# byu-magicc/VI-EKF

Hardware: AMD Instinct MI355X
Metric: EKF steps/sec (IMU-rate propagate + N_feat updates), batch=1024, N_feat=50 (higher is better)
Workload: dtype f64

## Files before the change

vi_ekf_amd/csrc/viekf_resident_common.hpp:

```cpp
#pragma once
#include <type_traits>

#include "viekf_fused_lds.hpp"
#include "viekf_instance_rows.hpp"
#include "viekf_kernel_args.hpp"

namespace viekf {

#ifndef RES_INLINE
#define RES_INLINE __forceinline__
#endif
__device__ __forceinline__ void wave_lds_sync() {
  __builtin_amdgcn_fence(__ATOMIC_RELEASE, "wavefront");
  __builtin_amdgcn_wave_barrier();
  __builtin_amdgcn_fence(__ATOMIC_ACQUIRE, "wavefront");
}
__device__ __forceinline__ int opaque(int v) { asm volatile("" : "+v"(v)); return v; }
typedef double v2f64 __attribute__((ext_vector_type(2)));
__device__ __forceinline__ double2 lds_ld2(const double* p) {
  const v2f64 v = *reinterpret_cast<const v2f64*>(p);
  return make_double2(v.x, v.y);
}
template <bool ON>
__device__ __forceinline__ void group_fence() {
  if (ON) {
    asm volatile("" ::: "memory");
    __builtin_amdgcn_sched_barrier(0);
  }
}
__device__ __forceinline__ double uniform_f64(double v) {
  const unsigned long long u = __double_as_longlong(v);
  const unsigned lo = __builtin_amdgcn_readfirstlane((unsigned)u), hi = __builtin_amdgcn_readfirstlane((unsigned)(u >> 32));
  return __longlong_as_double(((unsigned long long)hi << 32) | lo);
}

#ifdef VIEKF_STAMPS
#if VIEKF_STAMPS + 0 == 2
#define RES_STAMP_KEPT(idx) ((idx) >= 192 && (idx) < 224)
#else
#define RES_STAMP_KEPT(idx) true
#endif
#define RES_STAMP(S_, who, idx)                                                                  \
  do {                                                                                           \
    if (RES_STAMP_KEPT(idx) && (S_).b == 0 && (who)) {                                                                  \
      __builtin_amdgcn_sched_barrier(0);                                                         \
      reinterpret_cast<unsigned long long*>((S_).stamps)[(idx)] = __builtin_amdgcn_s_memtime();  \
      __builtin_amdgcn_sched_barrier(0);                                                         \
    }                                                                                            \
  } while (0)
#else
#define RES_STAMP(S_, who, idx) do {} while (0)
#endif

#ifdef VIEKF_ISA_MARKS
#define RES_MARK(name)                          \
  do {                                          \
    __builtin_amdgcn_sched_barrier(0);          \
    asm volatile("; @@MARK " name);             \
    __builtin_amdgcn_sched_barrier(0);          \
  } while (0)
#else
#define RES_MARK(name) do {} while (0)
#endif

#ifdef VIEKF_ABLATE
#define RES_ABLATE(S_, bit) (((S_).dbg & (bit)) != 0)
#else
#define RES_ABLATE(S_, bit) false
#endif

typedef __attribute__((address_space(3))) volatile int lds_vint_t;

struct ResShared {
  double *xs, *Kt, *Wt, *Praw, *lam, *sm, *fixadd, *fixset, *Z, *phiff, *Abb, *Gb, *Phibb, *Mbb, *Gdb, *Pbb, *T16,
      *xdb, *Pbc, *PhibbT, *Pd, *PsiP, *Pi, *Xi, *AvG, *Lbc, *mz, *mR;
  int* mslot;
  int2* mseq;
  BodyCtx* ctx;
  int N, n, nf, len, M, mstride, do_prop, b, dbg, kp, B, img_len, mcap;
  int fmt;
  long si, so;
  double* stamps;
};

template <int RB, int TW>
__device__ __forceinline__ void res_words(const int* __restrict__ resmap, int t, int (&w)[RB]) {
#pragma unroll
  for (int ia = 0; ia < RB; ia++) w[ia] = resmap[ia * TW + t];
}
constexpr bool res_setup_under_load(int RB, int NW, bool MP) {
  return res_batched_loads(RB, NW) && !MP && ((NW == 3 && (RB == 4 || RB == 6 || RB == 7)) || (NW == 6 && RB == 5));
}
#ifndef VIEKF_SERVICE_SETUP
#define VIEKF_SERVICE_SETUP 1
#endif
#ifndef VIEKF_SERVICE_SETUP_CHUNKS
#define VIEKF_SERVICE_SETUP_CHUNKS 1
#endif
constexpr bool res_service_setup(int RB, int NW, bool MP) {
  return (VIEKF_SERVICE_SETUP) != 0 && res_setup_under_load(RB, NW, MP) && RB != 4;
}
#ifndef VIEKF_ROTATING_READS
#define VIEKF_ROTATING_READS 3
#endif
constexpr int res_rotating_reads(int RB, int NW, bool MP, bool ZU) {
  return (RB > 4) ? ((VIEKF_ROTATING_READS) & 3) : 0;
}
__device__ __forceinline__ bool res_word_blk(int e, int& I, int& J) {
  I = e & 0xff;
  J = (e >> 8) & 0xff;
  return (e >> 16) != 0;
}

__device__ __forceinline__ int res_next_valid(const ResShared& S, int from) {
  int m = from;
  while (m < S.M && S.mslot[m] < 0) m++;
  return m;
}

}
```

vi_ekf_amd/csrc/viekf_resident_worker.hpp:

```cpp
#pragma once
#include "viekf_resident_prop.hpp"

namespace viekf {


struct StoreChunk { int f0, f1, rb, h; };
__device__ __forceinline__ bool store_chunk_at(int f0, int N, int n, int img_len, StoreChunk& c) {
  if (f0 >= N) return false;
  c.f0 = f0;
  c.rb = (16 + 3 * f0) & ~1;
  c.h = ((n + 1) & ~1) - c.rb;
  c.f1 = min(N, f0 + max(1, img_len / (3 * c.h)));
  return true;
}
template <int T>
__device__ __forceinline__ void res_store_chunk(const StreamArgs& a, const ResShared& S, const StoreChunk& c, int tid) {
  const int n = S.n, ld = a.ld;
  double* P = a.P_out + S.so * n * ld;
  const double* img = S.Z;
  const int ncol = 3 * (c.f1 - c.f0), lane = tid & 63, w = tid >> 6;
  constexpr int NWV = T / 64;
  if ((n & 1) == 0) {
#pragma unroll 2
    for (int col = w; col < ncol; col += NWV) {
      const int j = 16 + 3 * c.f0 + col;
      const double* src = img + col * c.h - c.rb;
      for (int i0 = c.rb; i0 < n; i0 += 256) {
        double2 v[2];
#pragma unroll
        for (int u = 0; u < 2; u++) v[u] = lds_ld2(src + min(i0 + 2 * (lane + 64 * u), n - 2));
#pragma unroll
        for (int u = 0; u < 2; u++) {
          const int i = i0 + 2 * (lane + 64 * u);
          if (i < n && i + 1 >= j) *reinterpret_cast<double2*>(P + i + (long)j * ld) = v[u];
        }
      }
    }
  } else {
#pragma unroll 2
    for (int col = w; col < ncol; col += NWV) {
      const int j = 16 + 3 * c.f0 + col;
      const double* src = img + col * c.h - c.rb;
      for (int i = c.rb + lane; i < n; i += 64)
        if (i >= j) P[i + (long)j * ld] = src[i];
    }
  }
}

template <int RB, int TW>
__device__ __forceinline__ void res_store_packed(double* img, const double (&pb)[RB][9], const double* Pbc, const double* Pbb,
                                                 int N, int t) {
  constexpr ResPack K(0, RB, TW / 64);
  v2f64* dst = reinterpret_cast<v2f64*>(img) + t;
#pragma unroll
  for (int p = 0; p < K.npair; p++) {
    v2f64 v;
    v.x = pb[(2 * p) / 9][(2 * p) % 9];
    v.y = pb[(2 * p + 1) / 9][(2 * p + 1) % 9];
    dst[p * TW] = v;
  }
  if ((9 * RB) & 1) img[K.single + t] = pb[RB - 1][8];
  v2f64* gc = reinterpret_cast<v2f64*>(img + K.pbc);
  for (int e = t; e < 24 * N; e += TW) gc[e] = *reinterpret_cast<const v2f64*>(Pbc + 2 * e);
  v2f64* gb = reinterpret_cast<v2f64*>(img + K.pbc + 48 * N);
  for (int e = t; e < 128; e += TW) gb[e] = *reinterpret_cast<const v2f64*>(Pbb + 2 * e);
}
__device__ __forceinline__ void res_body_items(const ResShared& S, const double* kP, bool run, int id, int nthreads,
                                               int first, int last, int slot2, double* rawdst) {
  const double* wP = kP + 2 * S.n;
  double* Pbc = S.Pbc;
  const int j2 = ((first + id) & 7) * 2;
  double2 cw0 = {}, cw1 = {}, cl[3] = {};
  if (run) {
    cw0 = lds_ld2(wP + 2 * j2);
    cw1 = lds_ld2(wP + 2 * j2 + 2);
#pragma unroll
    for (int q = 0; q < 3; q++) cl[q] = lds_ld2(S.Lbc + 16 * q + j2);
  }
#pragma unroll 1
  for (int item = first + id; item < last; item += nthreads) {
    const int g = item >> 3;
    double2 cpv[3];
#pragma unroll
    for (int q = 0; q < 3; q++) cpv[q] = lds_ld2(Pbc + (3 * g + q) * 16 + j2);
    if (run) {
      double2 cki[3];
#pragma unroll
      for (int q = 0; q < 3; q++) cki[q] = lds_ld2(kP + 2 * (16 + 3 * g + q));
#pragma unroll
      for (int q = 0; q < 3; q++) {
        cpv[q].x = fma(-cl[q].x, fma(cki[q].y, cw0.y, cki[q].x * cw0.x), cpv[q].x);
        cpv[q].y = fma(-cl[q].y, fma(cki[q].y, cw1.y, cki[q].x * cw1.x), cpv[q].y);
        *reinterpret_cast<double2*>(Pbc + (3 * g + q) * 16 + j2) = cpv[q];
      }
    }
    if (g == slot2) {
      double* st = rawdst + 2 * j2;
      *reinterpret_cast<double2*>(st) = make_double2(cpv[0].x, cpv[1].x);
      *reinterpret_cast<double2*>(st + 2) = make_double2(cpv[0].y, cpv[1].y);
    }
  }
}
template <int RB, int TW, bool MP, int T = TW + 64, bool ZU = false, bool BL = true>
__device__ __forceinline__ void res_worker(const StreamArgs& a, const ResShared& S, int tid) {
  constexpr bool SU = res_setup_under_load(RB, TW / 64, MP);
  constexpr int RR = res_rotating_reads(RB, TW / 64, MP, ZU);
  const int N = S.N, n = S.n, ld = a.ld, nf = S.nf, len = S.len;
  double* P = a.P + S.si * n * ld;
  const int tid_ = tid;
  constexpr int NWV = TW / 64;
  const DevParams& prm = *a.dp;
  double* Pbc = S.Pbc;
  double* Pbb = S.Pbb;
  const int* __restrict__ resmap = a.resmap;
  auto blk = [&](const int (&w)[RB], int t, int ia, int& I, int& J) -> bool {
    return res_word_blk(BL ? w[ia] : resmap[ia * TW + t], I, J);
  };
  const bool own_diag = tid_ < N;

  double pb[RB][9];
  const bool ldp = (S.fmt & RES_FMT_LOAD_PACKED) != 0;
  double Lff[9];
  bool partial_su = false;
  if (SU) {
    const double lf[3] = {a.lambda[16], a.lambda[17], a.lambda[18]};
#pragma unroll
    for (int r = 0; r < 3; r++)
#pragma unroll
      for (int s = 0; s < 3; s++) Lff[r * 3 + s] = uniform_f64(prm.use_partial_update ? (lf[s] + lf[r] - lf[r] * lf[s]) : 1.0);
    partial_su = prm.use_partial_update != 0;
  }
  if (ldp) {
    const int t = opaque(tid_);
    constexpr ResPack K(0, RB, TW / 64);
    const v2f64* gc = reinterpret_cast<const v2f64*>(P + K.pbc);
    for (int e = t; e < 24 * N; e += TW) *reinterpret_cast<v2f64*>(Pbc + 2 * e) = gc[e];
    const v2f64* gb = reinterpret_cast<const v2f64*>(P + K.pbc + 48 * N);
    for (int e = t; e < 128; e += TW) *reinterpret_cast<v2f64*>(Pbb + 2 * e) = gb[e];
  }
  if (SU) {
    for (int e = tid; !ldp && e < nf * 16; e += TW) {
      const int k = e / nf, row = e - k * nf;
      Pbc[row * 16 + k] = P[(16 + row) + (long)k * ld];
    }
    for (int e = tid; !ldp && e < 256; e += TW) {
      const int r = e & 15, c = e >> 4;
      Pbb[r * 16 + c] = P[max(r, c) + (long)min(r, c) * ld];
    }
  }
  int ws[SU ? RB : 1];
  double qs[3];
  {
    const int tq = opaque(tid_);
    int ew[RB];
    if (BL) res_words<RB, TW>(resmap, tq, ew);
    if (SU) {
#pragma unroll
      for (int ia = 0; ia < RB; ia++) ws[ia] = ew[ia];
      if (S.do_prop) {
#pragma unroll
        for (int r = 0; r < 3; r++) qs[r] = a.Qx[16 + 3 * min(tq, N - 1) + r];
      }
    }
#pragma unroll
    for (int ia = 0; ia < (SU ? RB / 4 : RB); ia++) {
      int I, J;
      blk(ew, tq, ia, I, J);
      const bool up = I < J;
      const int br = 16 + 3 * (up ? J : I), bc = 16 + 3 * (up ? I : J);
      const unsigned cbase = (unsigned)(br + bc * ld);
      const unsigned base = ldp ? 2u * (unsigned)tq : cbase, base1 = ldp ? (unsigned)tq : cbase;
#pragma unroll
      for (int s = 0; s < 3; s++)
#pragma unroll
        for (int r = 0; r < 3; r++) {
          const int rr = (I == J) ? max(r, s) : (up ? s : r), cc = (I == J) ? min(r, s) : (up ? r : s);
          constexpr ResPack K(0, RB, TW / 64);
          const int q = ia * 9 + r * 3 + s;
          const unsigned offp = (unsigned)K.elem(q, 0), offc = (unsigned)(rr + cc * ld);
          pb[ia][r * 3 + s] = P[((q < 2 * K.npair) ? base : base1) + (ldp ? offp : offc)];
        }
    }
    for (int e = tid; !SU && !ldp && e < nf * 16; e += TW) {
      const int k = e / nf, row = e - k * nf;
      Pbc[row * 16 + k] = P[(16 + row) + (long)k * ld];
    }
    for (int e = tid; !SU && !ldp && e < 256; e += TW) {
      const int r = e & 15, c = e >> 4;
      Pbb[r * 16 + c] = P[max(r, c) + (long)min(r, c) * ld];
    }
  }

  auto issue_chunk = [&](auto kc) {
    constexpr int k = decltype(kc)::value + 1, lo = RB * k / 4, hi = RB * (k + 1) / 4;
    const int tq = opaque(tid_);
#pragma unroll
    for (int ia = lo; ia < hi; ia++) {
      int I, J;
      res_word_blk(ws[SU ? ia : 0], I, J);
      const bool up = I < J;
      const int br = 16 + 3 * (up ? J : I), bc = 16 + 3 * (up ? I : J);
      const unsigned cbase = (unsigned)(br + bc * ld);
      const unsigned base = ldp ? 2u * (unsigned)tq : cbase, base1 = ldp ? (unsigned)tq : cbase;
#pragma unroll
      for (int s = 0; s < 3; s++)
#pragma unroll
        for (int r = 0; r < 3; r++) {
          const int rr = (I == J) ? max(r, s) : (up ? s : r), cc = (I == J) ? min(r, s) : (up ? r : s);
          constexpr ResPack K(0, RB, TW / 64);
          const int q = ia * 9 + r * 3 + s;
          const unsigned offp = (unsigned)K.elem(q, 0), offc = (unsigned)(rr + cc * ld);
          pb[ia][r * 3 + s] = P[((q < 2 * K.npair) ? base : base1) + (ldp ? offp : offc)];
        }
    }
  };

  auto sym_diag = [&]() {
    if (own_diag) { pb[0][3] = pb[0][1]; pb[0][6] = pb[0][2]; pb[0][7] = pb[0][5]; }
  };
  if (!SU) {
    sym_diag();
    const double lf[3] = {a.lambda[16], a.lambda[17], a.lambda[18]};
#pragma unroll
    for (int r = 0; r < 3; r++)
#pragma unroll
      for (int s = 0; s < 3; s++) Lff[r * 3 + s] = uniform_f64(prm.use_partial_update ? (lf[s] + lf[r] - lf[r] * lf[s]) : 1.0);
  }
  const bool partial = SU ? partial_su : prm.use_partial_update != 0;
  int par = 0;
  constexpr int NSV = (T - TW) / 64;
  auto fix_word = [&](int mb) -> double { return (NSV > 1) ? S.sm[res_sm::fix_word(1, mb)] + S.sm[res_sm::fix_word(2, mb)] : S.sm[res_sm::fix_word(0, mb)]; };
  RES_STAMP(S, tid == 0, 64);
  __syncthreads();
  RES_STAMP(S, tid == 0, 65);

  const int nkp = MP ? S.kp : 1;
  int eu[RB];
  if (S.do_prop)
   for (int kp = 0; kp < nkp; kp++) {
    const int tk = MP ? opaque(tid) : tid;
    const double* Z = S.Z; double* phiff = S.phiff;
    int ep[RB];
    double qd[3];
    if (SU) {
#pragma unroll
      for (int ia = 0; ia < RB; ia++) ep[ia] = ws[SU ? ia : 0];
#pragma unroll
      for (int r = 0; r < 3; r++) qd[r] = qs[r];
    } else if (BL) {
      const int tq = opaque(tid_);
      res_words<RB, TW>(resmap, tq, ep);
#pragma unroll
      for (int r = 0; r < 3; r++) qd[r] = a.Qx[16 + 3 * min(tq, N - 1) + r];
    }
    if (MP || !BL) res_prop_setup<TW>(a, S, tk);
    else if (SU) res_prop_setup<TW, true, decltype(issue_chunk), res_service_setup(RB, TW / 64, MP)>(a, S, tk, issue_chunk);
    else res_prop_setup<TW, true>(a, S, tk);
    RES_STAMP(S, tid == 0, 66);
    __syncthreads();
    RES_STAMP(S, tid == 0, 67);
#ifdef VIEKF_STAMPS
    asm volatile("s_waitcnt vmcnt(0)" ::: "memory");
#endif
    RES_STAMP(S, tid == 0, 74);
    if (SU) sym_diag();

#pragma unroll
    for (int ia = 0; ia < RB; ia++) {
      const int tq = BL ? 0 : opaque(tid_);
      int I, J;
      const bool v = blk(ep, tq, ia, I, J);
      const double* fj = phiff + 9 * J;
#pragma unroll
      for (int r = 0; r < 3; r++) {
        const double p0 = pb[ia][r * 3 + 0], p1 = pb[ia][r * 3 + 1], p2 = pb[ia][r * 3 + 2];
#pragma unroll
        for (int s = 0; s < 3; s++) pb[ia][r * 3 + s] = p0 * fj[s * 3 + 0] + p1 * fj[s * 3 + 1] + p2 * fj[s * 3 + 2];
      }
      const double* fi = phiff + 9 * I;
#pragma unroll
      for (int s = 0; s < 3; s++) {
        const double p0 = pb[ia][0 * 3 + s], p1 = pb[ia][1 * 3 + s], p2 = pb[ia][2 * 3 + s];
#pragma unroll
        for (int r = 0; r < 3; r++) pb[ia][r * 3 + s] = fi[r * 3 + 0] * p0 + fi[r * 3 + 1] * p1 + fi[r * 3 + 2] * p2;
      }
      if (BL) {
        if (ia == 0 && own_diag) { pb[0][0] += qd[0]; pb[0][4] += qd[1]; pb[0][8] += qd[2]; }
      } else if (v && I == J) {
        pb[ia][0] += a.Qx[16 + 3 * I + 0];
        pb[ia][4] += a.Qx[16 + 3 * I + 1];
        pb[ia][8] += a.Qx[16 + 3 * I + 2];
      }
      __builtin_amdgcn_sched_barrier(0);
      if (RB > 4) {
#pragma unroll
        for (int e = 0; e < 9; e++) asm volatile("" : "+v"(pb[ia][e]));
      }
      group_fence<(RB > 4)>();
    }
    RES_STAMP(S, tid == 0, 68);
    int zoff[RB];
    {
      const int tq = BL ? 0 : opaque(tid_);
#pragma unroll
      for (int ia = 0; ia < RB; ia++) {
        int I, J;
        blk(ep, tq, ia, I, J);
        zoff[ia] = (3 * I * ZS) | ((3 * J * ZS) << 16);
      }
    }
    auto contract = [&](int k, auto crossed) {
      constexpr bool CROSS = decltype(crossed)::value;
      if (RR & 2) {
        double2 xb[2][3], yb[2][3];
#pragma unroll
        for (int ia = 0; ia < 2; ia++) {
          const double* zi = Z + (zoff[ia] & 0xffff) + 2 * k;
          const double* zj = Z + (zoff[ia] >> 16) + 2 * k;
#pragma unroll
          for (int r = 0; r < 3; r++) xb[ia][r] = lds_ld2(zi + r * ZS);
#pragma unroll
          for (int s = 0; s < 3; s++) yb[ia][s] = lds_ld2(zj + s * ZS);
        }
#pragma unroll
        for (int ia = 0; ia < RB; ia++) {
          const int ib = ia & 1;
#pragma unroll
          for (int r = 0; r < 3; r++)
#pragma unroll
            for (int s = 0; s < 3; s++) {
              double acc = pb[ia][r * 3 + s];
              acc = fma(xb[ib][r].x, CROSS ? yb[ib][s].y : yb[ib][s].x, acc);
              acc = fma(xb[ib][r].y, CROSS ? yb[ib][s].x : yb[ib][s].y, acc);
              pb[ia][r * 3 + s] = acc;
            }
          group_fence<true>();
          if (ia + 2 < RB) {
            constexpr int RBL = RB - 1;
            const int in = (ia + 2 < RB) ? ia + 2 : RBL;
            const double* zi = Z + (zoff[in] & 0xffff) + 2 * k;
            const double* zj = Z + (zoff[in] >> 16) + 2 * k;
#pragma unroll
            for (int r = 0; r < 3; r++) xb[ib][r] = lds_ld2(zi + r * ZS);
#pragma unroll
            for (int s = 0; s < 3; s++) yb[ib][s] = lds_ld2(zj + s * ZS);
          }
        }
        return;
      }
#pragma unroll
      for (int ia = 0; ia < RB; ia++) {
        const double* zi = Z + (zoff[ia] & 0xffff) + 2 * k;
        const double* zj = Z + (zoff[ia] >> 16) + 2 * k;
        double2 xv[3], yv[3];
#pragma unroll
        for (int r = 0; r < 3; r++) xv[r] = lds_ld2(zi + r * ZS);
#pragma unroll
        for (int s = 0; s < 3; s++) yv[s] = lds_ld2(zj + s * ZS);
#pragma unroll
        for (int r = 0; r < 3; r++)
#pragma unroll
          for (int s = 0; s < 3; s++) {
            double acc = pb[ia][r * 3 + s];
            acc = fma(xv[r].x, CROSS ? yv[s].y : yv[s].x, acc);
            acc = fma(xv[r].y, CROSS ? yv[s].x : yv[s].y, acc);
            pb[ia][r * 3 + s] = acc;
          }
        if (ia & 1) group_fence<(RB > 4)>();
      }
    };
#pragma unroll 1
    for (int k = 0; k < ZK; k++) contract(k, std::true_type{});
#pragma unroll 1
    for (int k = ZK; k < ZK + 3; k++) contract(k, std::false_type{});
    sym_diag();
    RES_STAMP(S, tid == 0, 69);
    if (BL && !MP) res_words<RB, TW>(resmap, opaque(tid_), eu);
    if (MP) res_prop_body<TW, BL>(a, S, tk);
    par ^= 1;
    RES_STAMP(S, tid == 0, 70);
    __syncthreads();
    for (int e = tk; e < 256; e += TW) { const int r = e >> 4, c = e & 15; Pbb[e] = S.Mbb[min(r, c) * 16 + max(r, c)]; }
    if (MP && kp + 1 < nkp && own_diag && tid_ < len && fix_word(par ^ 1) != 0.0) {
      const int mb = par ^ 1, I = tid_;
      const double ad = S.fixadd[mb * N + I], st = S.fixset[mb * N + I];
      if (ad != 0.0) { pb[0][8] += ad; S.fixadd[mb * N + I] = 0.0; }
      if (st != 0.0) { pb[0][8] = prm.P0_feat[2]; S.fixset[mb * N + I] = 0.0; }
    }
   }

  if (SU && !S.do_prop) {
    issue_chunk(std::integral_constant<int, 0>{});
    issue_chunk(std::integral_constant<int, 1>{});
    issue_chunk(std::integral_constant<int, 2>{});
    sym_diag();
  }
  int Ib[RB], Jb[RB];
  bool vb[RB];
  if (BL && (MP || !S.do_prop)) res_words<RB, TW>(resmap, opaque(tid_), eu);
#pragma unroll
  for (int ia = 0; ia < RB; ia++) vb[ia] = blk(eu, tid_, ia, Ib[ia], Jb[ia]);
  const double p0rr = uniform_f64(prm.P0_feat[2]);
  auto bb_mask = [&](int r, int c) -> double { const double lr_ = S.lam[r], lc_ = S.lam[c]; return partial ? (lc_ + lr_ - lr_ * lc_) : 1.0; };
  double bbL0 = 1.0, bbL1 = 1.0;
  {
    constexpr int BBT0 = (TW >= 128) ? 128 : TW;
    const int ib0 = tid - (TW - BBT0);
    if (ib0 >= 0 && ib0 < 128) { bbL0 = bb_mask(ib0 >> 3, (ib0 & 7) * 2); bbL1 = bb_mask(ib0 >> 3, (ib0 & 7) * 2 + 1); }
  }
  auto apply_fixes = [&](int mb, double pending) {
    if (pending == 0.0) return;
    if (own_diag && tid_ < len) {
      VIEKF_COLD_BEGIN();
      const int I = tid_;
      const double ad = S.fixadd[mb * N + I], st = S.fixset[mb * N + I];
      if (ad != 0.0) { pb[0][8] += ad; S.fixadd[mb * N + I] = 0.0; }
      if (st != 0.0) { pb[0][8] = p0rr; S.fixset[mb * N + I] = 0.0; }
      VIEKF_COLD_END();
    }
  };
  auto extract_cols = [&](int slot, double* Pw) {
#pragma unroll
    for (int ia = 0; ia < RB; ia++) {
      const int I = Ib[ia], J = Jb[ia];
      const bool asrow = J == slot;
      const bool ascol = !asrow && I == slot;
      if (vb[ia] && (asrow || ascol)) {
        const int base = 16 + 3 * (asrow ? I : J);
        const double a0 = pb[ia][0], a1 = asrow ? pb[ia][1] : pb[ia][3];
        const double b0 = asrow ? pb[ia][3] : pb[ia][1], b1 = pb[ia][4];
        const double c0 = asrow ? pb[ia][6] : pb[ia][2], c1 = asrow ? pb[ia][7] : pb[ia][5];
        *reinterpret_cast<double2*>(Pw + 2 * (base + 0)) = make_double2(a0, a1);
        *reinterpret_cast<double2*>(Pw + 2 * (base + 1)) = make_double2(b0, b1);
        *reinterpret_cast<double2*>(Pw + 2 * (base + 2)) = make_double2(c0, c1);
      }
    }
  };

  int m = res_next_valid(S, 0);
  if (own_diag) {
    *reinterpret_cast<double2*>(S.Pd + 4 * tid_) = make_double2(pb[0][0], pb[0][1]);
    *reinterpret_cast<double2*>(S.Pd + 4 * tid_ + 2) = make_double2(pb[0][3], pb[0][4]);
  }
  int2 sq = S.mseq[min(m, S.mcap - 1)];
  if (m < S.M) {
    apply_fixes(par ^ 1, fix_word(par ^ 1));
    const int s0 = S.mslot[m];
    extract_cols(s0, S.Praw);
    if (sq.y >= 0) extract_cols(sq.y, S.Praw + 2 * n);
    const int e = opaque(tid);
    if (e < 16) {
      const int sf = (e < 8) ? s0 : sq.y, ijj = (e & 7) * 2;
      if (sf >= 0) {
        const double2 q0 = lds_ld2(Pbc + (3 * sf) * 16 + ijj);
        const double2 q1 = lds_ld2(Pbc + (3 * sf + 1) * 16 + ijj);
        double* d = S.Praw + ((e < 8) ? 0 : 2 * n) + 2 * ijj;
        *reinterpret_cast<double2*>(d) = make_double2(q0.x, q1.x);
        *reinterpret_cast<double2*>(d + 2) = make_double2(q0.y, q1.y);
      }
    }
  }
  RES_STAMP(S, tid == 0, 71);
  __syncthreads();
  __syncthreads();
  int it_ = 0;
  int cnt = 0;
  while (m < S.M) {
    const int mnext = sq.x;
    RES_MARK("worker.phase_top");
    const double* kP = (cnt & 1) ? S.Z : S.Kt;
    const double* wP = kP + 2 * n;
    __builtin_amdgcn_s_setprio(1);
    const double fixpending = fix_word(par ^ 1);
    const double gflag = S.sm[res_sm::gate_word(cnt)];
    const double nanw = (NSV > 1) ? S.sm[res_sm::nan_word(1, cnt)] + S.sm[res_sm::nan_word(2, cnt)] : S.sm[res_sm::nan_word(0, cnt)];
    sq = S.mseq[min(mnext, S.mcap - 1)];
    RES_STAMP(S, tid == 0 && it_ < 8, 80 + 4 * it_ + 1);
    RES_STAMP(S, (tid & 63) == 0 && it_ == 3, 192 + 4 * (tid >> 6) + 0);
    const int it = tid;
    constexpr int GB = (RB <= 4) ? RB : 2;
    RES_MARK("worker.block_sweep");
    const bool gated = gflag != 0.0;
    const bool run = !gated && nanw == 0.0 && !RES_ABLATE(S, 1);
    bool fixed = false;
    if (RR & 1) {
      apply_fixes(par ^ 1, fixpending);
      if (run) {
        double2 kb[2][3], wb[2][3];
#pragma unroll
        for (int ia = 0; ia < 2; ia++) {
#pragma unroll
          for (int r = 0; r < 3; r++) kb[ia][r] = lds_ld2(kP + 2 * (16 + 3 * Ib[ia] + r));
#pragma unroll
          for (int s = 0; s < 3; s++) wb[ia][s] = lds_ld2(wP + 2 * (16 + 3 * Jb[ia] + s));
        }
#pragma unroll
        for (int ia = 0; ia < RB; ia++) {
          const int ib = ia & 1;
#pragma unroll
          for (int r = 0; r < 3; r++)
#pragma unroll
            for (int s = 0; s < 3; s++) {
              if (ZU && !(r == 2 && s == 2)) {
                pb[ia][r * 3 + s] = fma(-kb[ib][r].y, wb[ib][s].y, fma(-kb[ib][r].x, wb[ib][s].x, pb[ia][r * 3 + s]));
              } else {
                const double t = fma(kb[ib][r].y, wb[ib][s].y, kb[ib][r].x * wb[ib][s].x);
                pb[ia][r * 3 + s] = fma(-Lff[r * 3 + s], t, pb[ia][r * 3 + s]);
              }
            }
          group_fence<true>();
          if (ia + 2 < RB) {
            constexpr int RBL = RB - 1;
            const int in = (ia + 2 < RB) ? ia + 2 : RBL;
#pragma unroll
            for (int r = 0; r < 3; r++) kb[ib][r] = lds_ld2(kP + 2 * (16 + 3 * Ib[in] + r));
#pragma unroll
            for (int s = 0; s < 3; s++) wb[ib][s] = lds_ld2(wP + 2 * (16 + 3 * Jb[in] + s));
          }
        }
      }
    } else
#pragma unroll
    for (int g0 = 0; g0 < RB; g0 += GB) {
      double2 kI[GB][3], wJ[GB][3];
#pragma unroll
      for (int ig = 0; ig < GB; ig++) {
        const int ia = (g0 + ig < RB) ? g0 + ig : RB - 1;
#pragma unroll
        for (int r = 0; r < 3; r++) kI[ig][r] = lds_ld2(kP + 2 * (16 + 3 * Ib[ia] + r));
#pragma unroll
        for (int s = 0; s < 3; s++) wJ[ig][s] = lds_ld2(wP + 2 * (16 + 3 * Jb[ia] + s));
      }
      if (!fixed) { apply_fixes(par ^ 1, fixpending); fixed = true; }
      if (run) {
#pragma unroll
        for (int ig = 0; ig < GB; ig++) {
          if (g0 + ig >= RB) continue;
          const int ia = g0 + ig;
#pragma unroll
          for (int r = 0; r < 3; r++)
#pragma unroll
            for (int s = 0; s < 3; s++) {
              if (ZU && !(r == 2 && s == 2)) {
                pb[ia][r * 3 + s] = fma(-kI[ig][r].y, wJ[ig][s].y, fma(-kI[ig][r].x, wJ[ig][s].x, pb[ia][r * 3 + s]));
              } else {
                const double t = fma(kI[ig][r].y, wJ[ig][s].y, kI[ig][r].x * wJ[ig][s].x);
                pb[ia][r * 3 + s] = fma(-Lff[r * 3 + s], t, pb[ia][r * 3 + s]);
              }
            }
        }
      }
      group_fence<(RB > GB)>();
    }
    sym_diag();
    RES_MARK("worker.column_extraction");
    RES_STAMP(S, tid == 0 && it_ < 8, 160 + 4 * it_ + 0);
    double* rawdst = S.Praw + (cnt & 1) * 2 * n;
    if (sq.y >= 0 && !RES_ABLATE(S, 4) && !(RES_ABLATE(S, 8) && (cnt & 1))) extract_cols(sq.y, rawdst);
    __builtin_amdgcn_s_setprio(0);
    RES_STAMP(S, tid == 0 && it_ < 8, 160 + 4 * it_ + 1);
    RES_STAMP(S, (tid & 63) == 0 && it_ == 3, 192 + 4 * (tid >> 6) + 2);
    __builtin_amdgcn_sched_barrier(0);
    RES_MARK("worker.body_items");
    res_body_items(S, kP, run, (it >= 64) ? it - 64 : it + TW - 64, TW, 0, 8 * N, sq.y, rawdst);
    RES_MARK("worker.body_block");
    if (run) {
      constexpr int BBT = (TW >= 128) ? 128 : TW;
#pragma unroll
      for (int ib = it - (TW - BBT); ib >= 0 && ib < 128; ib += BBT) {
        const int br = ib >> 3, bc2 = (ib & 7) * 2;
        double2 bpv = *reinterpret_cast<double2*>(Pbb + br * 16 + bc2);
        const double2 kr = lds_ld2(kP + 2 * br), wr = lds_ld2(wP + 2 * br);
        const double2 k0 = lds_ld2(kP + 2 * bc2), w0 = lds_ld2(wP + 2 * bc2);
        const double2 k1 = lds_ld2(kP + 2 * bc2 + 2), w1 = lds_ld2(wP + 2 * bc2 + 2);
        const double L0 = (BBT == 128) ? bbL0 : bb_mask(br, bc2), L1 = (BBT == 128) ? bbL1 : bb_mask(br, bc2 + 1);
        const bool up0 = br <= bc2, up1 = br <= bc2 + 1;
        const double2 ka = up0 ? kr : k0, wa = up0 ? w0 : wr;
        const double2 kb = up1 ? kr : k1, wb = up1 ? w1 : wr;
        bpv.x = fma(-L0, fma(ka.y, wa.y, ka.x * wa.x), bpv.x);
        bpv.y = fma(-L1, fma(kb.y, wb.y, kb.x * wb.x), bpv.y);
        *reinterpret_cast<double2*>(Pbb + br * 16 + bc2) = bpv;
      }
    }
    RES_MARK("worker.phase_tail");
    par ^= 1;
    cnt++;
    RES_STAMP(S, tid == 0 && it_ < 8, 80 + 4 * it_ + 2);
    RES_STAMP(S, (tid & 63) == 0 && it_ == 3, 192 + 4 * (tid >> 6) + 1);
    __syncthreads();
    RES_STAMP(S, tid == 0 && it_ < 8, 80 + 4 * it_ + 3);
    RES_STAMP(S, (tid & 63) == 0 && it_ == 3, 192 + 4 * (tid >> 6) + 3);
    it_++;
    m = mnext;
  }
  RES_MARK("worker.loop_end");
  apply_fixes(par ^ 1, fix_word(par ^ 1));
  RES_STAMP(S, tid == 0, 72);
  __syncthreads();

  P = a.P_out + S.so * n * ld;
  if (S.fmt & RES_FMT_STORE_PACKED) {
    res_store_packed<RB, TW>(P, pb, Pbc, Pbb, N, opaque(tid_));
  } else {
    int es[RB];
    if (BL) res_words<RB, TW>(resmap, opaque(tid_), es);
    for (int e = opaque(tid); e < nf * 16; e += TW) {
      const int k = e / nf, row = e - k * nf;
      P[(16 + row) + (long)k * ld] = Pbc[row * 16 + k];
    }
    for (int e = opaque(tid); e < 256; e += TW) P[(e >> 4) + (long)(e & 15) * ld] = Pbb[e];
    double* img = S.Z;
    const int gtid = threadIdx.x;
    RES_STAMP(S, tid == 0, 224);
    StoreChunk sc;
    int ch = 0;
    for (int f0 = 0; store_chunk_at(f0, N, n, S.img_len, sc); f0 = sc.f1, ch++) {
      const int f1 = sc.f1;
      const int tq = BL ? 0 : opaque(tid_);
#pragma unroll
      for (int ia = 0; ia < RB; ia++) {
        int I, J;
        if (blk(es, tq, ia, I, J)) {
          if (I >= J && J >= f0 && J < f1) {
            double* d = img + (3 * (J - f0)) * sc.h + (16 + 3 * I - sc.rb);
#pragma unroll
            for (int s = 0; s < 3; s++)
#pragma unroll
              for (int r = 0; r < 3; r++) d[s * sc.h + r] = pb[ia][r * 3 + s];
          }
          if (I < J && I >= f0 && I < f1) {
            double* d = img + (3 * (I - f0)) * sc.h + (16 + 3 * J - sc.rb);
#pragma unroll
            for (int r = 0; r < 3; r++)
#pragma unroll
              for (int s = 0; s < 3; s++) d[r * sc.h + s] = pb[ia][r * 3 + s];
          }
        }
      }
      RES_STAMP(S, tid == 0 && ch < 3, 225 + 4 * ch);
      __syncthreads();
      RES_STAMP(S, tid == 0 && ch < 3, 226 + 4 * ch);
      res_store_chunk<T>(a, S, sc, gtid);
      RES_STAMP(S, tid == 0 && ch < 3, 227 + 4 * ch);
      __syncthreads();
      RES_STAMP(S, tid == 0 && ch < 3, 228 + 4 * ch);
    }
  }
  RES_STAMP(S, tid == 0, 73);
}


}
```

Before: 3.531 million.

## Software-pipeline LDS reads across block sweep and body-item phases in resident worker

For the RB=7, three-wave, non-MP configuration, this adds a phase-reads path that issues the first K/W gain LDS loads before the gate and NaN checks. Inside the block sweep it double-buffers the next block's K/W operands while the current block is updated. It also restructures body-item processing into a ping-pong loop that prefetches the next item's Pbc and K values, and issues the first item's reads before column extraction. The goal is to hide LDS latency behind FMAs, at the cost of extra registers for the duplicated buffers and more fences constraining the scheduler.

Measured after the change: 3.454 million. -2.2%, worse.

```diff
diff --git a/vi_ekf_amd/csrc/viekf_resident_common.hpp b/vi_ekf_amd/csrc/viekf_resident_common.hpp
--- a/vi_ekf_amd/csrc/viekf_resident_common.hpp
+++ b/vi_ekf_amd/csrc/viekf_resident_common.hpp
@@ -106,6 +106,12 @@
 constexpr int res_rotating_reads(int RB, int NW, bool MP, bool ZU) {
   return (RB > 4) ? ((VIEKF_ROTATING_READS) & 3) : 0;
 }
+#ifndef VIEKF_PHASE_READS
+#define VIEKF_PHASE_READS 3
+#endif
+constexpr int res_phase_reads(int RB, int NW, bool MP, bool ZU) {
+  return (!MP && RB == 7 && NW == 3 && (res_rotating_reads(RB, NW, MP, ZU) & 1)) ? ((VIEKF_PHASE_READS) & 3) : 0;
+}
 __device__ __forceinline__ bool res_word_blk(int e, int& I, int& J) {
   I = e & 0xff;
   J = (e >> 8) & 0xff;
diff --git a/vi_ekf_amd/csrc/viekf_resident_worker.hpp b/vi_ekf_amd/csrc/viekf_resident_worker.hpp
--- a/vi_ekf_amd/csrc/viekf_resident_worker.hpp
+++ b/vi_ekf_amd/csrc/viekf_resident_worker.hpp
@@ -105,6 +105,7 @@
 __device__ __forceinline__ void res_worker(const StreamArgs& a, const ResShared& S, int tid) {
   constexpr bool SU = res_setup_under_load(RB, TW / 64, MP);
   constexpr int RR = res_rotating_reads(RB, TW / 64, MP, ZU);
+  constexpr int PR = res_phase_reads(RB, TW / 64, MP, ZU);
   const int N = S.N, n = S.n, ld = a.ld, nf = S.nf, len = S.len;
   double* P = a.P + S.si * n * ld;
   const int tid_ = tid;
@@ -475,6 +476,18 @@
     const double gflag = S.sm[res_sm::gate_word(cnt)];
     const double nanw = (NSV > 1) ? S.sm[res_sm::nan_word(1, cnt)] + S.sm[res_sm::nan_word(2, cnt)] : S.sm[res_sm::nan_word(0, cnt)];
     sq = S.mseq[min(mnext, S.mcap - 1)];
+    double2 kb1[2][3], wb1[2][3];
+    if constexpr ((PR & 1) != 0) {
+      group_fence<true>();
+#pragma unroll
+      for (int ia = 0; ia < 2; ia++) {
+#pragma unroll
+        for (int r = 0; r < 3; r++) kb1[ia][r] = lds_ld2(kP + 2 * (16 + 3 * Ib[ia] + r));
+#pragma unroll
+        for (int s = 0; s < 3; s++) wb1[ia][s] = lds_ld2(wP + 2 * (16 + 3 * Jb[ia] + s));
+      }
+      group_fence<true>();
+    }
     RES_STAMP(S, tid == 0 && it_ < 8, 80 + 4 * it_ + 1);
     RES_STAMP(S, (tid & 63) == 0 && it_ == 3, 192 + 4 * (tid >> 6) + 0);
     const int it = tid;
@@ -483,7 +496,35 @@
     const bool gated = gflag != 0.0;
     const bool run = !gated && nanw == 0.0 && !RES_ABLATE(S, 1);
     bool fixed = false;
-    if (RR & 1) {
+    if constexpr ((PR & 1) != 0) {
+      apply_fixes(par ^ 1, fixpending);
+      if (run) {
+#pragma unroll
+        for (int ia = 0; ia < RB; ia++) {
+          const int ib = ia & 1;
+#pragma unroll
+          for (int r = 0; r < 3; r++)
+#pragma unroll
+            for (int s = 0; s < 3; s++) {
+              if (ZU && !(r == 2 && s == 2)) {
+                pb[ia][r * 3 + s] = fma(-kb1[ib][r].y, wb1[ib][s].y, fma(-kb1[ib][r].x, wb1[ib][s].x, pb[ia][r * 3 + s]));
+              } else {
+                const double t = fma(kb1[ib][r].y, wb1[ib][s].y, kb1[ib][r].x * wb1[ib][s].x);
+                pb[ia][r * 3 + s] = fma(-Lff[r * 3 + s], t, pb[ia][r * 3 + s]);
+              }
+            }
+          group_fence<true>();
+          if (ia + 2 < RB) {
+            constexpr int RBL = RB - 1;
+            const int in = (ia + 2 < RB) ? ia + 2 : RBL;
+#pragma unroll
+            for (int r = 0; r < 3; r++) kb1[ib][r] = lds_ld2(kP + 2 * (16 + 3 * Ib[in] + r));
+#pragma unroll
+            for (int s = 0; s < 3; s++) wb1[ib][s] = lds_ld2(wP + 2 * (16 + 3 * Jb[in] + s));
+          }
+        }
+      }
+    } else if (RR & 1) {
       apply_fixes(par ^ 1, fixpending);
       if (run) {
         double2 kb[2][3], wb[2][3];
@@ -556,6 +597,73 @@
     RES_MARK("worker.column_extraction");
     RES_STAMP(S, tid == 0 && it_ < 8, 160 + 4 * it_ + 0);
     double* rawdst = S.Praw + (cnt & 1) * 2 * n;
+    if constexpr ((PR & 2) != 0) {
+      static_assert(TW >= 128, "the body block's 128 tasks sit on the top 128 worker threads");
+      const int itq = opaque(it), last = 8 * N, slot2 = sq.y;
+      int item = (itq >= 64) ? itq - 64 : itq + TW - 64;
+      const int j2 = (item & 7) * 2;
+      double2 ca[3], cka[3], cb[3], ckb[3];
+      auto rd = [&](int i, double2 (&pv)[3], double2 (&ki)[3]) {
+        const int g = min(i, last - 1) >> 3;
+#pragma unroll
+        for (int q = 0; q < 3; q++) pv[q] = lds_ld2(Pbc + (3 * g + q) * 16 + j2);
+#pragma unroll
+        for (int q = 0; q < 3; q++) ki[q] = lds_ld2(kP + 2 * (16 + 3 * g + q));
+      };
+      const double2 cw0 = lds_ld2(wP + 2 * j2), cw1 = lds_ld2(wP + 2 * j2 + 2);
+      double2 cl[3];
+#pragma unroll
+      for (int q = 0; q < 3; q++) cl[q] = lds_ld2(S.Lbc + 16 * q + j2);
+      rd(item, ca, cka);
+      group_fence<true>();
+      if (sq.y >= 0 && !RES_ABLATE(S, 4) && !(RES_ABLATE(S, 8) && (cnt & 1))) extract_cols(sq.y, rawdst);
+      __builtin_amdgcn_s_setprio(0);
+      RES_STAMP(S, tid == 0 && it_ < 8, 160 + 4 * it_ + 1);
+      RES_STAMP(S, (tid & 63) == 0 && it_ == 3, 192 + 4 * (tid >> 6) + 2);
+      __builtin_amdgcn_sched_barrier(0);
+      RES_MARK("worker.body_items");
+      auto fin = [&](int i, double2 (&pv)[3], const double2 (&ki)[3]) {
+        const int g = i >> 3;
+        if (run) {
+#pragma unroll
+          for (int q = 0; q < 3; q++) {
+            pv[q].x = fma(-cl[q].x, fma(ki[q].y, cw0.y, ki[q].x * cw0.x), pv[q].x);
+            pv[q].y = fma(-cl[q].y, fma(ki[q].y, cw1.y, ki[q].x * cw1.x), pv[q].y);
+            *reinterpret_cast<double2*>(Pbc + (3 * g + q) * 16 + j2) = pv[q];
+          }
+        }
+        if (g == slot2) {
+          double* st = rawdst + 2 * j2;
+          *reinterpret_cast<double2*>(st) = make_double2(pv[0].x, pv[1].x);
+          *reinterpret_cast<double2*>(st + 2) = make_double2(pv[0].y, pv[1].y);
+        }
+      };
+#pragma unroll 1
+      while (item < last) {
+        rd(item + TW, cb, ckb);
+        group_fence<true>();
+        fin(item, ca, cka);
+        group_fence<true>();
+        item += TW;
+        if (item >= last) break;
+        rd(item + TW, ca, cka);
+        group_fence<true>();
+        fin(item, cb, ckb);
+        group_fence<true>();
+        item += TW;
+      }
+      RES_MARK("worker.body_block");
+      if (run && itq >= TW - 128) {
+        const int ibb = itq - (TW - 128), br = ibb >> 3, bc2 = (ibb & 7) * 2;
+        const bool up0 = br <= bc2, up1 = br <= bc2 + 1;
+        double2 bpv = lds_ld2(Pbb + br * 16 + bc2);
+        const double2 bka = lds_ld2(kP + 2 * (up0 ? br : bc2)), bwa = lds_ld2(wP + 2 * (up0 ? bc2 : br));
+        const double2 bkb = lds_ld2(kP + 2 * (up1 ? br : bc2 + 1)), bwb = lds_ld2(wP + 2 * (up1 ? bc2 + 1 : br));
+        bpv.x = fma(-bbL0, fma(bka.y, bwa.y, bka.x * bwa.x), bpv.x);
+        bpv.y = fma(-bbL1, fma(bkb.y, bwb.y, bkb.x * bwb.x), bpv.y);
+        *reinterpret_cast<double2*>(Pbb + br * 16 + bc2) = bpv;
+      }
+    } else {
     if (sq.y >= 0 && !RES_ABLATE(S, 4) && !(RES_ABLATE(S, 8) && (cnt & 1))) extract_cols(sq.y, rawdst);
     __builtin_amdgcn_s_setprio(0);
     RES_STAMP(S, tid == 0 && it_ < 8, 160 + 4 * it_ + 1);
@@ -582,6 +690,7 @@
         *reinterpret_cast<double2*>(Pbb + br * 16 + bc2) = bpv;
       }
     }
+    }
     RES_MARK("worker.phase_tail");
     par ^= 1;
     cnt++;
```
